# nhcha6/embodied-object-detection

Measured on AMD Instinct MI355X. Metric: frames/sec (640x640, implicit_memory); frames/sec/GPU = value / n_gpus, higher is better.
Workload: dtype f32

## Files before the change

embodied_object_detection_amd/csrc/conv_fp32.hip:

```cpp
#include "conv_operands.h"

namespace eodconv {
namespace {

template <int BM, int BN, int BK, bool TAP4, bool MULTI, int PIPE = 0>
__global__ __launch_bounds__(256) void conv_igemm_kernel(ConvArgs p) {
  constexpr bool BORDER = PIPE == 3;
  static_assert(!BORDER || (BM == 64 && BN == 64 && BK == 32 && !TAP4 && !MULTI), "border-major order: the plain 64x64 kernel");
  constexpr bool PF2 = PIPE == 1;
  constexpr bool DB = PIPE == 2;
  constexpr int LS = BK + 4;
  constexpr int TM = BM / 64, TN = BN / 64;
  constexpr int QPR = BK / 4;
  constexpr int RPP = 256 / QPR;
  constexpr int AR = BM / RPP, BR = BN / RPP;
  static_assert(!TAP4 || BK == 32, "the stem path stages one 7x7 tap per float4: BK must be 32");
  constexpr int BUF = (BM + BN) * LS;
  __shared__ __attribute__((aligned(16))) float lds[(DB ? 2 : 1) * BUF];
  float* As = lds;
  float* Bs = lds + BM * LS;

  const int tid = threadIdx.x;
  const int lane = tid & 63;
  const int wave = tid >> 6;
  const int wm = wave >> 1, wn = wave & 1;

  int M, tile_m, tile_n;
  if constexpr (BORDER) {
    if (!conv_claim_tile_border<BM>(p, M, tile_m, tile_n)) return;
  } else {
    const int t = conv_first_tile<BM>(p, M);
    if (t < 0) return;
    tile_m = t / p.tiles_n;
    tile_n = t - tile_m * p.tiles_n;
  }
  const int m0 = tile_m * BM, n0 = tile_n * BN;
  if (!conv_tile_active(p, m0, BM)) return;
  const int z = blockIdx.y;
  int c_end;
  const int c_begin = conv_chunk_range(p, p.cps, z, c_end);

  const int lr = tid / QPR, lq = tid % QPR;
  int a_off[AR], a_iy[AR], a_ix[AR];
  unsigned a_voff[AR];
  unsigned long long a_mask[AR];
  unsigned a_pitch[MULTI ? AR : 1];
  const int rois = BORDER ? border_rois(p) : 0;
#pragma unroll
  for (int i = 0; i < AR; ++i) {
    const int m = m0 + lr + RPP * i;
    const bool rowok = m < M;
    RowOrigin o;
    if constexpr (BORDER) o = conv_row_origin_border(p, m, rowok, rois);
    else o = conv_row_origin<MULTI>(p, m, rowok);
    a_iy[i] = rowok ? o.iy0 : -(1 << 28);
    a_ix[i] = o.ix0;
    a_off[i] = o.off;
    if (!TAP4) conv_row_address<MULTI>(p, o, rowok, lq, a_voff[i], a_mask[i], a_pitch[MULTI ? i : 0]);
  }
  unsigned w_voff[BR];
#pragma unroll
  for (int j = 0; j < BR; ++j) w_voff[j] = conv_w_row_offset(p, n0 + lr + RPP * j, lq);
  const __amdgpu_buffer_rsrc_t rsrc_x = conv_buffer(p.x, p.x_bytes);
  const __amdgpu_buffer_rsrc_t rsrc_w = conv_buffer(p.w, p.w_bytes);

  unsigned live = 0;
  if constexpr (BORDER) {
    unsigned mine = 0;
#pragma unroll
// ... 87 lines not shown
  auto stage_and_multiply = [&](auto& ar, auto& br, int next_chunk) {
#pragma unroll
    for (int i = 0; i < AR; ++i) *reinterpret_cast<f32x4*>(As + (lr + RPP * i) * LS + 4 * lq) = ar[i];
#pragma unroll
    for (int j = 0; j < BR; ++j) *reinterpret_cast<f32x4*>(Bs + (lr + RPP * j) * LS + 4 * lq) = br[j];
    __syncthreads();
    if (next_chunk < c_end) load_chunk(next_chunk, ar, br);
    if constexpr (TM * TN == 1) {
      f32x4 af[2], bf[2];
      af[0] = *reinterpret_cast<const f32x4*>(a_base);
      bf[0] = *reinterpret_cast<const f32x4*>(b_base);
#pragma unroll
      for (int kk = 0; kk < BK / 8; ++kk) {
        const int cur = kk & 1, nxt = cur ^ 1;
        if (kk + 1 < BK / 8) {
          af[nxt] = *reinterpret_cast<const f32x4*>(a_base + (kk + 1) * 8);
          bf[nxt] = *reinterpret_cast<const f32x4*>(b_base + (kk + 1) * 8);
        }
        __builtin_amdgcn_s_setprio(1);
#pragma unroll
        for (int tt = 0; tt < 4; ++tt)
          if (tt & 1)
            acc_b = __builtin_amdgcn_mfma_f32_32x32x2f32(af[cur][tt], bf[cur][tt], acc_b, 0, 0, 0);
          else
            acc[0][0] = __builtin_amdgcn_mfma_f32_32x32x2f32(af[cur][tt], bf[cur][tt], acc[0][0], 0, 0, 0);
        __builtin_amdgcn_s_setprio(0);
      }
    } else {
      multiply(a_base, b_base);
    }
    __syncthreads();
  };
  load_chunk(c_begin, ar0, br0);
  if constexpr (DB) {
    auto store_tiles = [&](int buf) {
#pragma unroll
      for (int i = 0; i < AR; ++i) *reinterpret_cast<f32x4*>(As + buf * BUF + (lr + RPP * i) * LS + 4 * lq) = ar0[i];
#pragma unroll
      for (int j = 0; j < BR; ++j) *reinterpret_cast<f32x4*>(Bs + buf * BUF + (lr + RPP * j) * LS + 4 * lq) = br0[j];
    };
    store_tiles(0);
    __syncthreads();
    int cur = 0;
    for (int chunk = c_begin; chunk < c_end; ++chunk) {
      const bool more = chunk + 1 < c_end;
      if (more) load_chunk(chunk + 1, ar0, br0);
      multiply(a_base + cur * BUF, b_base + cur * BUF);
      if (more) store_tiles(cur ^ 1);
      __syncthreads();
      cur ^= 1;
    }
  } else if constexpr (PF2) {
    if (c_begin + 1 < c_end) load_chunk(c_begin + 1, ar1, br1);
    for (int chunk = c_begin; chunk < c_end; chunk += 2) {
      stage_and_multiply(ar0, br0, chunk + 2);
      if (chunk + 1 < c_end) stage_and_multiply(ar1, br1, chunk + 3);
    }
  } else {
    for (int chunk = c_begin; chunk < c_end; ++chunk) stage_and_multiply(ar0, br0, chunk + 1);
  }

  if (TM * TN == 1) {
#pragma unroll
    for (int r = 0; r < 16; ++r) acc[0][0][r] += acc_b[r];
  }
  if constexpr (BM == 64 && BN == 256) {
    if (p.out_mode == 2) {
      float sred[16];
#pragma unroll
      for (int r = 0; r < 16; ++r) sred[r] = 0.f;
#pragma unroll
      for (int j = 0; j < TN; ++j) {
        const int co = (wn * TN + j) * 32 + (lane & 31);
        const float bw = p.bias ? p.bias[co] : 0.f;
        const float pw = p.fuse_w[co];
#pragma unroll
        for (int r = 0; r < 16; ++r) {
          float v = (acc[0][j][r] + bw) * p.out_scale;
          if (p.relu) v = fmaxf(v, 0.f);
          sred[r] += v * pw;
        }
      }
#pragma unroll
      for (int off = 16; off > 0; off >>= 1)
#pragma unroll
        for (int r = 0; r < 16; ++r) sred[r] += __shfl_xor(sred[r], off, 64);
      float* red = lds;
      if ((lane & 31) == 0) {
        const int half = lane >> 5;
#pragma unroll
        for (int r = 0; r < 16; ++r) red[(wm * 2 + wn) * 32 + (r & 3) + 8 * (r >> 2) + 4 * half] = sred[r];
      }
      __syncthreads();
      if (tid < BM) {
        const int wr = tid >> 5, rr = tid & 31;
        const float v = red[(wr * 2 + 0) * 32 + rr] + red[(wr * 2 + 1) * 32 + rr] + p.fuse_b;
        const int m = m0 + tid;
        if (m < M) {
          const int tq = (int)fdiv((unsigned)m, p.div_ow);
          const int ox = m - tq * p.OW;
          const int img = (int)fdiv((unsigned)tq, p.div_oh);
          const int oy = tq - img * p.OH;
          const int unit = p.out_units ? p.out_units[img] : img;
          const int dy = tile_n >> 1, dx = tile_n & 1;
          p.y[((size_t)unit * 2 * p.OH + 2 * oy + dy) * (2 * p.OW) + 2 * ox + dx] = eod_sigmoid_precise(v);
        }
      }
      return;
    }
  }
  store_wave_tiles<TM, TN, BM == 64 && BN == 64, BORDER>(p, acc, m0 + wm * TM * 32, n0 + wn * TN * 32, M, z, lane);
}


template <int NW, bool MULTI>
__global__ __launch_bounds__(NW * 64) void conv_wavek_kernel(ConvArgs p) {
  constexpr int BK = 32;
  constexpr int LS = BK + 4;
  constexpr int AR = 4;
  __shared__ __attribute__((aligned(16))) float lds[NW * 2 * 32 * LS];
  const int tid = threadIdx.x;
  const int lane = tid & 63;
  const int wave = tid >> 6;
  float* As = lds + wave * (2 * 32 * LS);
  float* Bs = As + 32 * LS;

  int M;
  const int t = conv_first_tile<32>(p, M);
  if (t < 0) return;
  const int tile_m = t / p.tiles_n;
  const int tile_n = t - tile_m * p.tiles_n;
  const int m0 = tile_m * 32, n0 = tile_n * 32;
  if (!conv_tile_active(p, m0, 32)) return;

  int c_end;
  const int c_begin = conv_chunk_range(p, (p.nchunks + NW - 1) / NW, wave, c_end);

  const int lr = lane >> 3, lq = lane & 7;
  unsigned a_voff[AR];
// ... 86 lines not shown
}

template <int BM, int BN>
static void launch_fp32_tile(const ConvArgs& a, bool tap4, int bk, dim3 grid, hipStream_t s, int dyn) {
  if (tap4)
    hipLaunchKernelGGL((conv_igemm_kernel<BM, BN, 32, true, false>), grid, dim3(256), dyn, s, a);
  else if (a.nlv > 0 && bk == 64)
    hipLaunchKernelGGL((conv_igemm_kernel<BM, BN, 64, false, true>), grid, dim3(256), dyn, s, a);
  else if (a.nlv > 0)
    hipLaunchKernelGGL((conv_igemm_kernel<BM, BN, 32, false, true>), grid, dim3(256), dyn, s, a);
  else if (bk == 64)
    hipLaunchKernelGGL((conv_igemm_kernel<BM, BN, 64, false, false>), grid, dim3(256), dyn, s, a);
  else
    hipLaunchKernelGGL((conv_igemm_kernel<BM, BN, 32, false, false>), grid, dim3(256), dyn, s, a);
}

void launch_conv_fp32(const ConvArgs& a, int tile, int bk, bool tap4, dim3 grid, hipStream_t s, int lds_reserve, int prefetch2) {
  const int dyn = lds_reserve > 0 ? lds_reserve : 0;
  if (a.border) {
    hipLaunchKernelGGL((conv_igemm_kernel<64, 64, 32, false, false, 3>), grid, dim3(256), dyn, s, a);
    return;
  }
  if (prefetch2 == 1 && !tap4 && a.nlv == 0 && bk == 32 && tile == 3) {
    hipLaunchKernelGGL((conv_igemm_kernel<64, 64, 32, false, false, 1>), grid, dim3(256), dyn, s, a);
    return;
  }
  if (prefetch2 == 2 && !tap4 && bk == 32 && tile == 3) {
    if (a.nlv > 0) hipLaunchKernelGGL((conv_igemm_kernel<64, 64, 32, false, true, 2>), grid, dim3(256), dyn, s, a);
    else hipLaunchKernelGGL((conv_igemm_kernel<64, 64, 32, false, false, 2>), grid, dim3(256), dyn, s, a);
    return;
  }
  switch (tile) {
    case 5: hipLaunchKernelGGL((conv_igemm_kernel<64, 256, 32, false, false>), grid, dim3(256), dyn, s, a); break;
    case 1: launch_fp32_tile<128, 128>(a, tap4, bk, grid, s, dyn); break;
    case 2: launch_fp32_tile<128, 64>(a, tap4, bk, grid, s, dyn); break;
    default: launch_fp32_tile<64, 64>(a, tap4, bk, grid, s, dyn); break;
  }
}

void launch_conv_wavek(const ConvArgs& a, int nw, dim3 grid, hipStream_t s) {
  if (a.nlv > 0) {
    if (nw == 8) hipLaunchKernelGGL((conv_wavek_kernel<8, true>), grid, dim3(512), 0, s, a);
    else hipLaunchKernelGGL((conv_wavek_kernel<4, true>), grid, dim3(256), 0, s, a);
  } else {
    if (nw == 8) hipLaunchKernelGGL((conv_wavek_kernel<8, false>), grid, dim3(512), 0, s, a);
    else hipLaunchKernelGGL((conv_wavek_kernel<4, false>), grid, dim3(256), 0, s, a);
  }
}

}
```

embodied_object_detection_amd/csrc/conv_igemm.hip:

```cpp
#include "conv_common.h"
#include "../../include/eod_hip.h"
#include <atomic>
#include <cstdlib>
#include <cstring>

namespace {

using namespace eodconv;

template <int VEC>
__global__ __launch_bounds__(256) void conv_splitk_reduce_kernel(ConvArgs p) {
  EOD_CHAIN_PRIO();
  const int M = conv_row_limit(p, p.M);
  const unsigned per_row = (unsigned)p.Cout / VEC;
  const unsigned total = (unsigned)M * per_row;
  const size_t slab = (size_t)p.M * p.Cout;
  for (unsigned idx = blockIdx.x * blockDim.x + threadIdx.x; idx < total; idx += gridDim.x * blockDim.x) {
    const unsigned m = fdiv(idx, p.div_row);
    if (!conv_row_active(p, (int)m)) continue;
    const unsigned n = (idx - m * per_row) * VEC;
    const float* src = p.partial + (size_t)m * p.Cout + n;
    if (VEC == 4) {
      f32x4 v = {0.f, 0.f, 0.f, 0.f};
      for (int zb = 0; zb < p.splitk; zb += 4) {
// ... 67 lines not shown
    red[sub][col / cpg4][0] = s;
    red[sub][col / cpg4][1] = q;
  }
  __syncthreads();
  if ((int)threadIdx.x < p.gn_groups) {
    double ts = 0.0, tq = 0.0;
    for (int u = 0; u < nsub; ++u) {
      ts += red[u][threadIdx.x][0];
      tq += red[u][threadIdx.x][1];
    }
    p.gn_partial[((size_t)blockIdx.x * p.gn_groups + threadIdx.x) * 2 + 0] = ts;
    p.gn_partial[((size_t)blockIdx.x * p.gn_groups + threadIdx.x) * 2 + 1] = tq;
  }
}

std::atomic<int>& math_mode() {
  static std::atomic<int> v([] {
    const char* e = getenv("EOD_CONV_MATH");
    if (e && strcmp(e, "bf16x3") == 0) return EOD_MATH_BF16X3;
    if (e && strcmp(e, "f16") == 0) return EOD_MATH_F16;
    return EOD_MATH_FP32;
  }());
  return v;
}

struct Plan {
  int tile;
  int bk;
  int glds;
  int bm, bn, tiles_m, tiles_n, splitk, cps, nchunks;
  int wavek;
  int pw_np;
  int border;
};

constexpr int kForcePointwise = 30;

int effective_math(const EodConvDesc* d) { return d->math > 0 ? d->math - 1 : math_mode().load(std::memory_order_relaxed); }

bool pointwise_eligible(const EodConvDesc* d) {
  return effective_math(d) == EOD_MATH_FP32 && d->KH == 1 && d->KW == 1 && d->stride == 1 && d->pad == 0 && d->levels <= 0 && !d->tap4 &&
         d->Cin == d->Kpad && (d->Cin == 64 || d->Cin == 128 || d->Cin == 256) && d->Cout % 64 == 0 && d->out_mode == 0 &&
         (d->res_mode == 0 || d->res_mode == 1) && !d->in_relu && !d->gate && !d->m_count && d->split_n == 0 && !d->gn_partial &&
         d->lds_reserve == 0;
}

constexpr int kForceBorder = 43;
constexpr bool kBorderAuto = true;

bool border_eligible(const EodConvDesc* d) {
  return effective_math(d) == EOD_MATH_FP32 && d->KH == 3 && d->KW == 3 && d->stride == 1 && d->pad == 1 && d->levels <= 0 && !d->tap4 &&
         d->m_count && d->m_segments <= 1 && d->m_unit == d->OH * d->OW && d->OH >= 3 && d->OW >= 3 && d->Cin % 32 == 0 &&
         d->out_mode == 0 && d->res_mode == 0 && !d->in_relu && !d->gate && d->split_n == 0 && !d->gn_partial && d->prefetch2 == 0;
}

Plan make_plan(const EodConvDesc* d, int M) {
  static const int cfg[5][2] = {{128, 128}, {128, 64}, {64, 64}, {256, 128}, {64, 256}};
  Plan pl{};
  int pick = 2;
  const int ft = d->force_tile % 10, fbk = d->force_tile / 10;
  const bool half_ok = !d->tap4 && !d->in_relu;
  const bool f16_forced = (fbk == 8 || fbk == 9) && half_ok;
  if (f16_forced) pick = ft == 4 ? 3 : 2;
  else if (ft >= 1 && ft <= 3) pick = ft - 1;
  else if (ft == 4 && fbk == 5 && half_ok) pick = 3;
  const bool bk64_ok = !d->tap4 && d->Cin % 64 == 0 && d->Kpad % 64 == 0;
  pl.glds = f16_forced ? 3 : ((fbk == 5 && half_ok) ? 2 : 0);
  const int Mp = (d->plan_rows > 0 && d->plan_rows < M) ? d->plan_rows : M;
  const int math = effective_math(d);
  if (d->force_tile == 0 && math == EOD_MATH_F16 && half_ok) {
    pl.glds = 3;
    pick = (long)((Mp + 255) / 256) * ((d->Cout + 127) / 128) >= 256 ? 3 : 2;
  }
  if (d->force_tile == 0 && math == EOD_MATH_BF16X3 && half_ok) {
    pl.glds = 2;
    const long t128 = (long)((Mp + 127) / 128) * ((d->Cout + 127) / 128);
    const long t256 = (long)((Mp + 255) / 256) * ((d->Cout + 127) / 128);
    pick = t256 >= 256 ? 3 : (t128 >= 512 ? 0 : 2);
  }
  if (d->out_mode == 2) {
    pick = 4;
    pl.glds = 0;
  }
  if (d->gate) {
    const bool f16_gated = d->math == EOD_MATH_F16 + 1 && half_ok && d->levels <= 0 && (d->force_tile == 0 || f16_forced);
    pick = 2;
    pl.glds = f16_gated ? 3 : 0;
  }
  if (pl.glds == 3) pl.bk = (fbk == 8 && d->Cin % 64 == 0) ? 64 : 32;
  else pl.bk = (pl.glds == 0 && d->out_mode != 2 && fbk == 2 && bk64_ok) ? 64 : 32;
  const int nchunks = d->Kpad / pl.bk;
  pl.nchunks = nchunks;
  pl.tile = pick + 1;
  pl.bm = cfg[pick][0];
  pl.bn = cfg[pick][1];
  pl.tiles_m = (M + pl.bm - 1) / pl.bm;
  pl.tiles_n = (d->Cout + pl.bn - 1) / pl.bn;
  const long tiles = (long)((Mp + pl.bm - 1) / pl.bm) * pl.tiles_n;
  int splitk = 1;
  if (d->out_mode == 2) {
    splitk = 1;
  } else if (d->force_splitk > 0) {
    splitk = d->force_splitk;
  } else if (pl.glds == 0 && !d->tap4 && nchunks >= 8 &&
             ((d->force_tile == 6 || d->force_tile == 7) ||
              (tiles < 256 && nchunks <= 192 && pl.bk == 32 && d->force_tile == 0 &&
               ((Mp <= 512 && nchunks / (nchunks >= 64 ? 8 : 4) >= 8) || nchunks >= 128)))) {
    pl.wavek = d->force_tile == 6 ? 4 : (d->force_tile == 7 ? 8 : (nchunks >= 64 ? 8 : 4));
    pl.bk = 32;
    pl.nchunks = d->Kpad / 32;
    pl.bm = pl.bn = 32;
    pl.tiles_m = (M + 31) / 32;
    pl.tiles_n = (d->Cout + 31) / 32;
  } else if (tiles < 256 && nchunks >= 8) {
    const int target = (nchunks >= 128 && Mp <= 512) ? 1792 : 512;
    int want = (int)((target + tiles - 1) / tiles);
    int maxs = nchunks / 4;
    splitk = want < maxs ? want : maxs;
    if (splitk < 1) splitk = 1;
  } else if (tiles >= 256 && tiles <= 1024 && d->m_count == nullptr && nchunks >= 18) {
    double best = 1e30;
    for (int sct = 1; sct <= 4; ++sct) {
      if (nchunks / sct < 9) break;
      const double est = (double)((tiles * sct + 255) / 256) / sct + (sct > 1 ? 0.12 : 0.0);
      if (est < best - 1e-9) {
        best = est;
        splitk = sct;
      }
    }
  }
// ... 62 lines not shown
    if (d->OW != (d->W + 2 * d->pad - d->KW) / d->stride + 1) return EOD_ERR_BAD_DIMS;
  }
  if (d->levels <= 0 && (long)d->N * d->H * d->W * d->Cin >= (1L << 29)) return EOD_ERR_BAD_DIMS;
  if ((long)d->Cout * d->Kpad >= (1L << 29)) return EOD_ERR_BAD_DIMS;
  if (d->KH * d->KW > 64) return EOD_ERR_BAD_DIMS;
  if ((long)total_rows(d) * (d->Cout > d->Cin ? d->Cout : d->Cin) >= (1L << 31)) return EOD_ERR_BAD_DIMS;
  if (d->out_mode == 1 && (d->Cout % 4 != 0)) return EOD_ERR_BAD_DIMS;
  if (d->out_mode == 2) {
    if (d->Cout != 1024 || d->KH != 1 || d->KW != 1 || d->stride != 1 || d->tap4 || d->levels > 0 || d->res_mode != 0 || d->in_relu ||
        d->force_splitk > 1)
      return EOD_ERR_BAD_DIMS;
    if (!d->fuse_w) return EOD_ERR_NULL;
  }
  if (d->out_mode < 0 || d->out_mode > 2) return EOD_ERR_BAD_DIMS;
  if (d->res_mode != 0 && !d->res) return EOD_ERR_NULL;
  if (d->res_mode == 2 && ((d->OH & 1) || (d->OW & 1))) return EOD_ERR_BAD_DIMS;
  if (d->m_count && d->m_unit <= 0) return EOD_ERR_BAD_DIMS;
  if (d->m_segments > 1) {
    if (!d->m_count || d->levels > 0 || d->out_mode == 2 || d->m_segments > EOD_MAX_BATCH || d->N % d->m_segments != 0)
      return EOD_ERR_BAD_DIMS;
    if (((long)(d->N / d->m_segments) * d->OH * d->OW) % d->m_unit != 0) return EOD_ERR_BAD_DIMS;
  }
  if (d->gate && (d->out_mode != 0 || d->split_n != 0 || d->gn_partial)) return EOD_ERR_BAD_DIMS;
  if (d->gate && d->force_tile != 0 && d->force_tile % 10 != 3 && d->force_tile != 6 && d->force_tile != 7) return EOD_ERR_BAD_DIMS;
  if (d->gate && d->force_tile / 10 == 5) return EOD_ERR_BAD_DIMS;
  if (d->gate && (d->force_tile / 10 == 8 || d->force_tile / 10 == 9) &&
      (d->math != EOD_MATH_F16 + 1 || d->force_tile % 10 != 3 || d->levels > 0 || d->tap4 || d->in_relu))
    return EOD_ERR_BAD_DIMS;
  if (d->math < 0 || d->math > EOD_MATH_F16 + 1) return EOD_ERR_BAD_DIMS;
  if ((d->force_tile / 10 == 8 || d->force_tile / 10 == 9) && d->force_tile % 10 != 3 && d->force_tile % 10 != 4) return EOD_ERR_BAD_DIMS;
  if (d->lds_reserve < 0 || d->lds_reserve > 48 * 1024) return EOD_ERR_BAD_DIMS;
  if (d->force_tile == kForcePointwise && (!pointwise_eligible(d) || d->force_splitk > 1)) return EOD_ERR_BAD_DIMS;
  if (d->force_tile == kForceBorder && (!border_eligible(d) || d->force_splitk > 1)) return EOD_ERR_BAD_DIMS;
  if (d->split_n != 0) {
    if (!d->y2) return EOD_ERR_NULL;
    if (d->split_n < 0 || d->split_n >= d->Cout || d->out_mode != 0 || d->res_mode != 0 || d->levels > 0 || d->gn_partial)
      return EOD_ERR_BAD_DIMS;
  }
  if (d->gn_partial) {
    const int cpg = d->gn_groups > 0 ? d->Cout / d->gn_groups : 0;
    if (d->levels <= 0 || d->m_count || d->out_mode != 0 || d->gn_groups <= 0 || d->gn_groups > 64 || d->Cout % d->gn_groups != 0 ||
        cpg > 64 || (cpg & (cpg - 1)) != 0 || cpg < 4 || d->Cout % 4 != 0 || d->Cout > 1024 || 256 % (d->Cout / 4) != 0 ||
        64 % (cpg / 4) != 0)
      return EOD_ERR_BAD_DIMS;
  }
  if (!eod_aligned16(d->x) || !eod_aligned16(d->w) || !eod_aligned16(d->w_split) || !eod_aligned16(d->w_half)) return EOD_ERR_ALIGN;
  return EOD_OK;
}

}

extern "C" int eod_set_conv_math(int mode) {
  if (mode != EOD_MATH_FP32 && mode != EOD_MATH_BF16X3 && mode != EOD_MATH_F16) return EOD_ERR_BAD_DIMS;
  return math_mode().exchange(mode);
}

extern "C" int eod_get_conv_math(void) { return math_mode().load(); }

extern "C" size_t eod_conv_split_weights_bytes(int Cout, int Kpad) {
  return (Cout > 0 && Kpad > 0 && Kpad % 32 == 0) ? (size_t)Cout * Kpad * 6 : 0;
}

extern "C" int eod_conv_split_weights_bf16x3(const float* w, int Cout, int Kpad, void* out, eod_stream_t stream) {
  if (!w || !out) return EOD_ERR_NULL;
  if (Cout <= 0 || Kpad <= 0 || Kpad % 32 != 0 || (long)Cout * Kpad * 6 >= (1L << 32)) return EOD_ERR_BAD_DIMS;
  if (!eod_aligned16(w) || !eod_aligned16(out)) return EOD_ERR_ALIGN;
// ... 70 lines not shown
    a.w3_bytes = (unsigned)((size_t)d->Cout * d->Kpad * 6);
    a.wh = d->w_half;
    a.wh_bytes = (unsigned)((size_t)d->Cout * d->Kpad * 2);
  }
  a.nlv = d->levels > 0 ? d->levels : 0;
  for (int l = 0; l < a.nlv; ++l) {
    a.lv_off[l] = d->level_off[l];
    a.lv_h[l] = d->level_h[l];
    a.lv_w[l] = d->level_w[l];
  }
  if (a.nlv) a.lv_off[a.nlv] = d->level_off[a.nlv];
  a.relu = d->relu; a.res_mode = d->res_mode; a.in_relu = d->in_relu; a.out_mode = d->out_mode;
  a.gate = d->gate;
  a.out_scale = d->out_scale;
  a.gn_partial = d->gn_partial;
  a.gn_groups = d->gn_groups;
  a.y2 = d->y2;
  a.split_n = d->split_n;
  const Plan pl = make_plan(d, a.M);
  if (d->gn_partial && pl.splitk <= 1) return EOD_ERR_BAD_DIMS;
  a.nchunks = pl.nchunks;
  a.splitk = pl.splitk; a.cps = pl.cps; a.tiles_m = pl.tiles_m; a.tiles_n = pl.tiles_n;
  a.border = pl.border;
  if (pl.splitk > 1) {
    const size_t need = (size_t)pl.splitk * a.M * a.Cout * sizeof(float);
    if (!d->workspace || d->workspace_bytes < need) return EOD_ERR_CAPACITY;
  }
  dim3 grid(pl.tiles_m * pl.tiles_n, pl.splitk);
  if (pl.border) grid.x = (pl.tiles_m + 7) / 8 * 8 * pl.tiles_n;
  if (pl.pw_np) launch_conv_pointwise(a, pl.pw_np, grid, s);
  else if (pl.wavek) launch_conv_wavek(a, pl.wavek, grid, s);
  else if (pl.glds == 3) launch_conv_f16(a, pl.tile, pl.bk, grid, s);
  else if (pl.glds == 2) launch_conv_bf16x3(a, pl.tile, grid, s);
  else launch_conv_fp32(a, pl.tile, pl.bk, d->tap4 != 0, grid, s, d->lds_reserve, d->prefetch2);
  if (pl.splitk > 1) {
    const size_t total = (size_t)a.M * a.Cout;
    const bool vec = a.Cout % 4 == 0;
    int blocks = (int)((total / (vec ? 4 : 1) + 255) / 256);
    if (blocks > 2048) blocks = 2048;
    if (blocks < 1) blocks = 1;
    if (a.gn_partial) {
      int chunks = 0;
      for (int l = 0; l < a.nlv; ++l) chunks += (a.lv_off[l + 1] - a.lv_off[l] + EOD_GN_ROWS - 1) / EOD_GN_ROWS;
      hipLaunchKernelGGL(conv_splitk_reduce_gn_kernel, dim3(chunks), dim3(256), 0, s, a);
    } else if (vec) hipLaunchKernelGGL(conv_splitk_reduce_kernel<4>, dim3(blocks), dim3(256), 0, s, a);
    else hipLaunchKernelGGL(conv_splitk_reduce_kernel<1>, dim3(blocks), dim3(256), 0, s, a);
  }
  return eod_launch_status();
}
```

embodied_object_detection_amd/modeling/roi_heads.py:

```python
from __future__ import annotations

from typing import Dict, List, Tuple

import torch

from .. import ops
from ..registry import ROI_HEADS_REGISTRY


RESULT_SETS = 3


class RoiBuffers:

    def __init__(self, heads: "DeticCascadeROIHeads", B: int, lockstep: bool):
        R, D, dev = heads.R, heads.topk, heads.device
        f32 = dict(dtype=torch.float32, device=dev)
        self.device, self.B, self.R, self.D, self.rows = dev, B, R, D, B * R
        self.lockstep = lockstep
        self.batch, self.m_segments = (B, B) if lockstep else (1, 0)
        self.plan_like_single = True
        self.pool7 = torch.empty((B * R, 7, 7, 256), **f32)
        self.h1 = torch.empty((B * R, 1, 1, 1024), **f32)
        self.h2 = torch.empty((B * R, 1, 1, 1024), **f32)
# ... 82 lines not shown
        self.stages = []
        for k in range(self.num_stages):
            fc1_w = sd[f"roi_heads.box_head.{k}.fc1.weight"]
            fc1_w = fc1_w.view(-1, 256, 7, 7).permute(0, 2, 3, 1).reshape(fc1_w.shape[0], -1, 1, 1).contiguous()
            p = f"roi_heads.box_predictor.{k}"
            st = dict(
                fc1=ops.Conv(fc1_w, sd[f"roi_heads.box_head.{k}.fc1.bias"], device=device, name=f"box_head.{k}.fc1"),
                fc2=ops.Conv(sd[f"roi_heads.box_head.{k}.fc2.weight"][:, :, None, None], sd[f"roi_heads.box_head.{k}.fc2.bias"],
                             device=device, name=f"box_head.{k}.fc2"),
                cls=ops.Conv(sd[f"{p}.cls_score.linear.weight"][:, :, None, None], sd[f"{p}.cls_score.linear.bias"], device=device,
                             name=f"box_predictor.{k}.cls_score.linear"),
                bb0=ops.Conv(sd[f"{p}.bbox_pred.0.weight"][:, :, None, None], sd[f"{p}.bbox_pred.0.bias"], device=device,
                             name=f"box_predictor.{k}.bbox_pred.0"),
                bb2=ops.Conv(sd[f"{p}.bbox_pred.2.weight"][:, :, None, None], sd[f"{p}.bbox_pred.2.bias"], device=device,
                             name=f"box_predictor.{k}.bbox_pred.2"),
                zs=sd[f"{p}.cls_score.zs_weight"].contiguous().to(device),
            )
            st["cls_bb0"] = ops.Conv(torch.cat([sd[f"{p}.cls_score.linear.weight"], sd[f"{p}.bbox_pred.0.weight"]], dim=0)[:, :, None, None],
                                     torch.cat([sd[f"{p}.cls_score.linear.bias"], sd[f"{p}.bbox_pred.0.bias"]], dim=0), device=device,
                                     name=f"box_predictor.{k}.cls_score.linear+bbox_pred.0")
            assert st["zs"].shape == (512, self.C1), (st["zs"].shape, self.C1)
            self.stages.append(st)
        m = "roi_heads.mask_head"
        self.mask_convs = [ops.Conv(sd[f"{m}.mask_fcn{i}.weight"], sd[f"{m}.mask_fcn{i}.bias"], pad=1, device=device, name=f"mask_fcn{i}")
                           for i in range(1, 5)]
        for conv in self.mask_convs:
            conv.prefetch2 = int(__import__("os").environ.get("EOD_MASK_PREFETCH2", "0"))
        self.deconv = ops.Conv(sd[f"{m}.deconv.weight"], sd[f"{m}.deconv.bias"], device=device, deconv=True, name="mask_deconv")
        self.pred_w = sd[f"{m}.predictor.weight"].reshape(-1).contiguous().to(device)
        self.pred_b = float(sd[f"{m}.predictor.bias"].item())
        self.bufs = RoiBuffers(self, 1, lockstep=False)
        self.bufs.expose_on(self)
        self.fuse_mask_tail = True
        self.merge_cls_bb0 = True
        self.fuse_stage_tail = True
        self.fold_deltas = False
        self.graph_cascade = False
        self._graphs = {}
        self.det_pass_lds_reserve = int(__import__("os").environ.get("EOD_DET_LDS_RESERVE", "0"))
        self.prop_pass_lds_reserve = int(__import__("os").environ.get("EOD_PROP_LDS_RESERVE", "0"))
        self.selectors = [ops.DetectionSelector(self.R, self.C1, self.topk, device, groups=True) for _ in range(RESULT_SETS)]
        self.selector = self.selectors[0]

    def set_classifier(self, zs: torch.Tensor) -> None:
        zs = zs.to(dtype=torch.float32).contiguous().to(self.device)
        if zs.dim() != 2 or zs.shape[0] != 512 or not 2 <= zs.shape[1] <= ops.ZS_WIDE_MAX_C1:
            raise ValueError(f"classifier matrix {tuple(zs.shape)}: expected [512, C + 1] with 1 <= C <= {ops.ZS_WIDE_MAX_C1 - 1}")
        for st in self.stages:
            st["zs"] = zs
        if zs.shape[1] != self.C1:
            self.C1 = int(zs.shape[1])
            self.num_classes = self.C1 - 1
            self.bufs.set_width(self.C1)
            self.bufs.expose_on(self)
            self.selectors = [ops.DetectionSelector(self.R, self.C1, self.topk, self.device, groups=True) for _ in range(RESULT_SETS)]
            self.selector = self.selectors[0]
        self._graphs = {}

    def forward_box(self, views: List[torch.Tensor], shapes, prop_boxes: torch.Tensor, prop_scores: torch.Tensor, count: torch.Tensor,
                    image_hw: Tuple[int, int], sel: int = 0, mem_rescore=None, after_stage0=None):
        h3, w3 = shapes[0]
        H, W = image_hw
        R = self.R
        if self.graph_cascade:
            key = (views[0].data_ptr(), prop_boxes.data_ptr(), prop_scores.data_ptr(), count.data_ptr(), mem_rescore is not None, H, W)
            gs = self._graphs.get(key)
# ... 68 lines not shown
                after_stage0()
            if not self.merge_cls_bb0:
                st["bb0"](g.h2, rows, 1, 1, relu=True, m_count=count, m_unit=1, out=g.hb, m_segments=segs, plan_rows=pr)
            st["bb2"](g.hb, rows, 1, 1, m_count=count, m_unit=1, out=g.deltas, m_segments=segs, plan_rows=pr)
            if self.fold_deltas and not last:
                pending = self.cascade_weights[k]
            else:
                ops.apply_deltas(g.deltas, 4, boxes, g.boxes[k + 1], count, R, self.cascade_weights[k], not last, float(W), float(H),
                                 batch=batch)
                boxes = g.boxes[k + 1]
        return boxes, pending

    def forward_mask(self, views, shapes, boxes: torch.Tensor, count: torch.Tensor, cap: int, out: torch.Tensor,
                     rows: torch.Tensor = None, bufs=None, lds_reserve: int = 0, tag=None, g: RoiBuffers = None,
                     boxes_per_image: int = 0):
        g = g if g is not None else self.bufs
        h3, w3 = shapes[0]
        mpool, mbuf, mup = bufs if bufs is not None else g.mask_bufs
        if not self.fuse_mask_tail and mup is None:
            raise NotImplementedError("fuse_mask_tail = False: the lock-step buffers hold no deconv output; run the two-launch mask tail "
                                      "on the single-scene model")
        cap, pr = g.B * cap, g.plan_rows(cap * 196)
        ops.roi_align(views[0], views[1], views[2], h3, w3, 256, boxes, count, cap, 14, out=mpool, box_rows=rows, batch=g.batch,
                      boxes_per_image=g.per_scene(boxes_per_image))
        src, dst = mpool, mbuf
        self.deconv.lds_reserve = lds_reserve
        for conv in self.mask_convs:
            conv.lds_reserve = lds_reserve
            conv.event_tag = tag
            conv(src, cap, 14, 14, relu=True, m_count=count, m_unit=196, out=dst, plan_rows=pr)
            src, dst = dst, src
        if self.fuse_mask_tail:
            self.deconv(src, cap, 14, 14, relu=True, m_count=count, m_unit=196, out=out, fuse=(self.pred_w, self.pred_b, rows),
                        plan_rows=pr)
        else:
            self.deconv(src, cap, 14, 14, relu=True, m_count=count, m_unit=196, out=mup, plan_rows=pr)
            ops.mask_predictor_sigmoid(mup, self.pred_w, self.pred_b, cap * 784, 256, count, 784, out=out, out_units=rows)
        return out

    def forward(self, views, shapes, prop_boxes, prop_scores, prop_count, image_hw):
        det = self.forward_box(views, shapes, prop_boxes, prop_scores, prop_count, image_hw)
        det_boxes, det_scores, det_classes, det_rows, det_count = det
        self.forward_mask(views, shapes, det_boxes, det_count, self.topk, self.det_masks)
        return det

    def forward_mask_memory(self, views, shapes, prop_boxes, prop_count, rows: torch.Tensor = None, rows_count: torch.Tensor = None,
                            bufs=None, tag=None, g: RoiBuffers = None, lds_reserve: int = None):
        g = g if g is not None else self.bufs
        lds = self.prop_pass_lds_reserve if lds_reserve is None else lds_reserve
        if rows is not None:
            rows, rows_count = g.roi_list(rows, rows_count, self.R)
            return self.forward_mask(views, shapes, prop_boxes, rows_count, min(self.R, 128), g.prop_masks, rows=rows, bufs=bufs,
                                     lds_reserve=lds, tag=tag, g=g, boxes_per_image=self.R)
        return self.forward_mask(views, shapes, prop_boxes, prop_count, self.R, g.prop_masks, bufs=bufs, lds_reserve=lds, tag=tag, g=g,
                                 boxes_per_image=self.R)

    def detection_masks(self, g: RoiBuffers, views, shapes, sel, slot: int, dedup: bool, lds_reserve: int, tag=None):
        rows, count = g.roi_list(sel.rep_list, sel.rep_count, self.topk, slot) if dedup else g.roi_list(None, sel.count, self.topk, slot)
        return self.forward_mask(views, shapes, sel.boxes, count, self.topk, g.det_masks, rows=rows, lds_reserve=lds_reserve, tag=tag,
                                 g=g, boxes_per_image=self.topk)

    def postprocess_and_paste(self, g: RoiBuffers, sel, post: dict, image_hw, mask_threshold: float, dedup: bool):
        H, W = image_hw
        B, D, dev = g.B, self.topk, self.device
        post["boxes"] = torch.empty((B * D, 4), dtype=torch.float32, device=dev)
        post["scores"] = torch.empty((B * D,), dtype=torch.float32, device=dev)
        post["classes"] = torch.empty((B * D,), dtype=torch.int32, device=dev)
# ... 13 lines not shown
```

embodied_object_detection_amd/ops.py:

```python
from __future__ import annotations

import ctypes as C
from typing import Dict, Optional, Sequence, Tuple

import numpy as np
import torch

from . import _lib
from ._lib import EodConvDesc, EodDetDesc, EodMemWriteDesc, EodProposalDesc, check


_raw_stream = getattr(torch._C, "_cuda_getCurrentRawStream", None)


def _stream() -> int:
    if _raw_stream is not None:
        return _raw_stream(torch.cuda.current_device())
    return torch.cuda.current_stream().cuda_stream


def _ptr(t: Optional[torch.Tensor]) -> Optional[int]:
    return None if t is None else t.data_ptr()


# ... 27 lines not shown
def set_conv_math(mode: str) -> str:
    if mode not in _CONV_MATH:
        hint = ""
        if str(mode).lower() == "fp16":
            hint = (' ("fp16" / FP16 is the config key of autocast training: modeling.training.build_trainer / AmpTrainer, which choose '
                    'the arithmetic per launch; the process-wide inference arithmetic is "f16")')
        raise ValueError(f"conv math must be one of {sorted(_CONV_MATH)}, got {mode!r}{hint}")
    prev = _lib.load().eod_set_conv_math(_CONV_MATH[mode])
    check(min(prev, 0), "eod_set_conv_math")
    return {v: k for k, v in _CONV_MATH.items()}[prev]


def get_conv_math() -> str:
    return {v: k for k, v in _CONV_MATH.items()}[_lib.load().eod_get_conv_math()]


def fold_bn(w: torch.Tensor, bn_w, bn_b, bn_mean, bn_var, eps: float = 1e-5):
    scale = bn_w / torch.sqrt(bn_var + eps)
    return w * scale.view(-1, 1, 1, 1), bn_b - bn_mean * scale


def pack_conv_weight(w_oihw: torch.Tensor, cin_pad: Optional[int] = None) -> Tuple[torch.Tensor, int]:
    O, I, KH, KW = w_oihw.shape
    w = w_oihw.permute(0, 2, 3, 1).contiguous()
    if cin_pad is not None and cin_pad != I:
        wp = torch.zeros((O, KH, KW, cin_pad), dtype=w.dtype)
        wp[..., :I] = w
        w = wp
    K = w.shape[1] * w.shape[2] * w.shape[3]
    Kpad = (K + 31) // 32 * 32
    out = torch.zeros((O, Kpad), dtype=torch.float32)
    out[:, :K] = w.reshape(O, K)
    return out.contiguous(), Kpad


class Conv:

    def __init__(self, w_oihw: torch.Tensor, bias: Optional[torch.Tensor], stride: int = 1, pad: int = 0,
                 device="cuda", cin_pad: Optional[int] = None, deconv: bool = False, name: str = ""):
        self.name = name
        if deconv:
            Cin, Cout, kh, kw = w_oihw.shape
            assert kh == 2 and kw == 2
            w = w_oihw.permute(2, 3, 1, 0).reshape(4 * Cout, Cin, 1, 1).contiguous()
            self.out_mode = 1
            self.KH = self.KW = 1
            self.stride, self.pad = 1, 0
            self.Cin, self.Cout = Cin, 4 * Cout
        else:
            w = w_oihw
            self.out_mode = 0
            self.Cout, cin, self.KH, self.KW = w.shape
            self.Cin = cin_pad or cin
            self.stride, self.pad = stride, pad
        packed, self.Kpad = pack_conv_weight(w, cin_pad)
        self.tap4 = 1 if self.Cin == 4 else 0
        if not self.tap4 and self.Cin % 32 != 0:
            raise ValueError(f"{name}: Cin={self.Cin} must be a multiple of 32 (or 4 for the stem)")
        self.w = packed.to(device)
        self.bias = None if bias is None else bias.detach().to(torch.float32).contiguous().to(device)
        self.desc = EodConvDesc()
        self._lib = _lib.load()
        self.w_split = None
        self.w_half = None
        self.event_log = None
        self.event_tag = None
# ... 1546 lines not shown
```

Before: 324.7.

## Split fused mask-tail deconv into two 128-wide passes per tile

```diff
diff --git a/embodied_object_detection_amd/csrc/conv_fp32.hip b/embodied_object_detection_amd/csrc/conv_fp32.hip
--- a/embodied_object_detection_amd/csrc/conv_fp32.hip
+++ b/embodied_object_detection_amd/csrc/conv_fp32.hip
@@ -2,10 +2,39 @@
 
 namespace eodconv {
 namespace {
+
+__device__ __forceinline__ void tail_chain(const ConvArgs& p, const f32x16& acc, int co, float (&sred)[16]) {
+  const float bw = p.bias ? p.bias[co] : 0.f;
+  const float pw = p.fuse_w[co];
+#pragma unroll
+  for (int r = 0; r < 16; ++r) {
+    float v = (acc[r] + bw) * p.out_scale;
+    if (p.relu) v = fmaxf(v, 0.f);
+    sred[r] = __builtin_fmaf(v, pw, sred[r]);
+  }
+}
+__device__ __forceinline__ void tail_butterfly(float (&sred)[16]) {
+#pragma unroll
+  for (int off = 16; off > 0; off >>= 1)
+#pragma unroll
+    for (int r = 0; r < 16; ++r) sred[r] += __shfl_xor(sred[r], off, 64);
+}
+__device__ __forceinline__ void tail_store(const ConvArgs& p, float v, int m, int tile_n) {
+  const int tq = (int)fdiv((unsigned)m, p.div_ow);
+  const int ox = m - tq * p.OW;
+  const int img = (int)fdiv((unsigned)tq, p.div_oh);
+  const int oy = tq - img * p.OH;
+  const int unit = p.out_units ? p.out_units[img] : img;
+  const int dy = tile_n >> 1, dx = tile_n & 1;
+  p.y[((size_t)unit * 2 * p.OH + 2 * oy + dy) * (2 * p.OW) + 2 * ox + dx] = eod_sigmoid_precise(v);
+}
 
 template <int BM, int BN, int BK, bool TAP4, bool MULTI, int PIPE = 0>
 __global__ __launch_bounds__(256) void conv_igemm_kernel(ConvArgs p) {
   constexpr bool BORDER = PIPE == 3;
+  constexpr bool TAIL2 = BM == 64 && BN == 128;
+  constexpr int NPASS = TAIL2 ? 2 : 1;
+  static_assert(!TAIL2 || (BK == 32 && !TAP4 && !MULTI && PIPE == 0), "two-pass tail: the default pipeline");
   static_assert(!BORDER || (BM == 64 && BN == 64 && BK == 32 && !TAP4 && !MULTI), "border-major order: the plain 64x64 kernel");
   constexpr bool PF2 = PIPE == 1;
   constexpr bool DB = PIPE == 2;
@@ -16,7 +45,8 @@
   constexpr int AR = BM / RPP, BR = BN / RPP;
   static_assert(!TAP4 || BK == 32, "the stem path stages one 7x7 tap per float4: BK must be 32");
   constexpr int BUF = (BM + BN) * LS;
-  __shared__ __attribute__((aligned(16))) float lds[(DB ? 2 : 1) * BUF];
+  constexpr int RED = TAIL2 ? 2 * 2 * 32 : 0;
+  __shared__ __attribute__((aligned(16))) float lds[(DB ? 2 : 1) * BUF + RED];
   float* As = lds;
   float* Bs = lds + BM * LS;
 
@@ -34,7 +64,7 @@
     tile_m = t / p.tiles_n;
     tile_n = t - tile_m * p.tiles_n;
   }
-  const int m0 = tile_m * BM, n0 = tile_n * BN;
+  const int m0 = tile_m * BM, n0 = tile_n * BN * NPASS;
   if (!conv_tile_active(p, m0, BM)) return;
   const int z = blockIdx.y;
   int c_end;
@@ -188,7 +218,53 @@
     __syncthreads();
   };
   load_chunk(c_begin, ar0, br0);
-  if constexpr (DB) {
+  if constexpr (TAIL2) {
+    float* hand = lds;
+    float* red = lds + BUF;
+#pragma nounroll
+    for (int pass = 0; pass < NPASS; ++pass) {
+      for (int chunk = c_begin; chunk < c_end; ++chunk) stage_and_multiply(ar0, br0, chunk + 1);
+      if (pass + 1 < NPASS) {
+#pragma unroll
+        for (int j = 0; j < BR; ++j) w_voff[j] = conv_w_row_offset(p, n0 + (pass + 1) * BN + lr + RPP * j, lq);
+        walk = ChunkWalker<BK, MULTI>(p, c_begin);
+        load_chunk(c_begin, ar0, br0);
+      }
+      float sred[16];
+      if (wn == 0) {
+#pragma unroll
+        for (int r = 0; r < 16; ++r) sred[r] = 0.f;
+#pragma unroll
+        for (int j = 0; j < TN; ++j) tail_chain(p, acc[0][j], pass * BN + j * 32 + (lane & 31), sred);
+#pragma unroll
+        for (int r = 0; r < 16; ++r) hand[(wm * 16 + r) * 64 + lane] = sred[r];
+      }
+      __syncthreads();
+      if (wn == 1) {
+#pragma unroll
+        for (int r = 0; r < 16; ++r) sred[r] = hand[(wm * 16 + r) * 64 + lane];
+#pragma unroll
+        for (int j = 0; j < TN; ++j) tail_chain(p, acc[0][j], pass * BN + (TN + j) * 32 + (lane & 31), sred);
+        tail_butterfly(sred);
+        if ((lane & 31) == 0) {
+          const int half = lane >> 5;
+#pragma unroll
+          for (int r = 0; r < 16; ++r) red[(pass * 2 + wm) * 32 + (r & 3) + 8 * (r >> 2) + 4 * half] = sred[r];
+        }
+      }
+      __syncthreads();
+#pragma unroll
+      for (int j = 0; j < TN; ++j)
+#pragma unroll
+        for (int r = 0; r < 16; ++r) acc[0][j][r] = 0.f;
+    }
+    if (tid < BM) {
+      const int wr = tid >> 5, rr = tid & 31;
+      const float v = red[(0 * 2 + wr) * 32 + rr] + red[(1 * 2 + wr) * 32 + rr] + p.fuse_b;
+      if (m0 + tid < M) tail_store(p, v, m0 + tid, tile_n);
+    }
+    return;
+  } else if constexpr (DB) {
     auto store_tiles = [&](int buf) {
 #pragma unroll
       for (int i = 0; i < AR; ++i) *reinterpret_cast<f32x4*>(As + buf * BUF + (lr + RPP * i) * LS + 4 * lq) = ar0[i];
@@ -226,21 +302,8 @@
 #pragma unroll
       for (int r = 0; r < 16; ++r) sred[r] = 0.f;
 #pragma unroll
-      for (int j = 0; j < TN; ++j) {
-        const int co = (wn * TN + j) * 32 + (lane & 31);
-        const float bw = p.bias ? p.bias[co] : 0.f;
-        const float pw = p.fuse_w[co];
-#pragma unroll
-        for (int r = 0; r < 16; ++r) {
-          float v = (acc[0][j][r] + bw) * p.out_scale;
-          if (p.relu) v = fmaxf(v, 0.f);
-          sred[r] += v * pw;
-        }
-      }
-#pragma unroll
-      for (int off = 16; off > 0; off >>= 1)
-#pragma unroll
-        for (int r = 0; r < 16; ++r) sred[r] += __shfl_xor(sred[r], off, 64);
+      for (int j = 0; j < TN; ++j) tail_chain(p, acc[0][j], (wn * TN + j) * 32 + (lane & 31), sred);
+      tail_butterfly(sred);
       float* red = lds;
       if ((lane & 31) == 0) {
         const int half = lane >> 5;
@@ -251,16 +314,7 @@
       if (tid < BM) {
         const int wr = tid >> 5, rr = tid & 31;
         const float v = red[(wr * 2 + 0) * 32 + rr] + red[(wr * 2 + 1) * 32 + rr] + p.fuse_b;
-        const int m = m0 + tid;
-        if (m < M) {
-          const int tq = (int)fdiv((unsigned)m, p.div_ow);
-          const int ox = m - tq * p.OW;
-          const int img = (int)fdiv((unsigned)tq, p.div_oh);
-          const int oy = tq - img * p.OH;
-          const int unit = p.out_units ? p.out_units[img] : img;
-          const int dy = tile_n >> 1, dx = tile_n & 1;
-          p.y[((size_t)unit * 2 * p.OH + 2 * oy + dy) * (2 * p.OW) + 2 * ox + dx] = eod_sigmoid_precise(v);
-        }
+        if (m0 + tid < M) tail_store(p, v, m0 + tid, tile_n);
       }
       return;
     }
@@ -413,6 +467,7 @@
   }
   switch (tile) {
     case 5: hipLaunchKernelGGL((conv_igemm_kernel<64, 256, 32, false, false>), grid, dim3(256), dyn, s, a); break;
+    case 7: hipLaunchKernelGGL((conv_igemm_kernel<64, 128, 32, false, false>), grid, dim3(256), dyn, s, a); break;
     case 1: launch_fp32_tile<128, 128>(a, tap4, bk, grid, s, dyn); break;
     case 2: launch_fp32_tile<128, 64>(a, tap4, bk, grid, s, dyn); break;
     default: launch_fp32_tile<64, 64>(a, tap4, bk, grid, s, dyn); break;
diff --git a/embodied_object_detection_amd/csrc/conv_igemm.hip b/embodied_object_detection_amd/csrc/conv_igemm.hip
--- a/embodied_object_detection_amd/csrc/conv_igemm.hip
+++ b/embodied_object_detection_amd/csrc/conv_igemm.hip
@@ -123,6 +123,7 @@
   int wavek;
   int pw_np;
   int border;
+  int tail2;
 };
 
 constexpr int kForcePointwise = 30;
@@ -138,6 +139,8 @@
 
 constexpr int kForceBorder = 43;
 constexpr bool kBorderAuto = true;
+
+constexpr int kForceTailWide = 45;
 
 bool border_eligible(const EodConvDesc* d) {
   return effective_math(d) == EOD_MATH_FP32 && d->KH == 3 && d->KW == 3 && d->stride == 1 && d->pad == 1 && d->levels <= 0 && !d->tap4 &&
@@ -187,6 +190,10 @@
   pl.bn = cfg[pick][1];
   pl.tiles_m = (M + pl.bm - 1) / pl.bm;
   pl.tiles_n = (d->Cout + pl.bn - 1) / pl.bn;
+  if (d->out_mode == 2 && d->force_tile != kForceTailWide) {
+    pl.tail2 = 1;
+    pl.bn = 128;
+  }
   const long tiles = (long)((Mp + pl.bm - 1) / pl.bm) * pl.tiles_n;
   int splitk = 1;
   if (d->out_mode == 2) {
@@ -315,6 +322,7 @@
   if (d->lds_reserve < 0 || d->lds_reserve > 48 * 1024) return EOD_ERR_BAD_DIMS;
   if (d->force_tile == kForcePointwise && (!pointwise_eligible(d) || d->force_splitk > 1)) return EOD_ERR_BAD_DIMS;
   if (d->force_tile == kForceBorder && (!border_eligible(d) || d->force_splitk > 1)) return EOD_ERR_BAD_DIMS;
+  if (d->force_tile == kForceTailWide && d->out_mode != 2) return EOD_ERR_BAD_DIMS;
   if (d->split_n != 0) {
     if (!d->y2) return EOD_ERR_NULL;
     if (d->split_n < 0 || d->split_n >= d->Cout || d->out_mode != 0 || d->res_mode != 0 || d->levels > 0 || d->gn_partial)
@@ -451,7 +459,7 @@
   else if (pl.wavek) launch_conv_wavek(a, pl.wavek, grid, s);
   else if (pl.glds == 3) launch_conv_f16(a, pl.tile, pl.bk, grid, s);
   else if (pl.glds == 2) launch_conv_bf16x3(a, pl.tile, grid, s);
-  else launch_conv_fp32(a, pl.tile, pl.bk, d->tap4 != 0, grid, s, d->lds_reserve, d->prefetch2);
+  else launch_conv_fp32(a, pl.tail2 ? 7 : pl.tile, pl.bk, d->tap4 != 0, grid, s, d->lds_reserve, d->prefetch2);
   if (pl.splitk > 1) {
     const size_t total = (size_t)a.M * a.Cout;
     const bool vec = a.Cout % 4 == 0;
diff --git a/embodied_object_detection_amd/modeling/roi_heads.py b/embodied_object_detection_amd/modeling/roi_heads.py
--- a/embodied_object_detection_amd/modeling/roi_heads.py
+++ b/embodied_object_detection_amd/modeling/roi_heads.py
@@ -138,6 +138,7 @@
         self.bufs = RoiBuffers(self, 1, lockstep=False)
         self.bufs.expose_on(self)
         self.fuse_mask_tail = True
+        self.mask_tail_force_tile = 0
         self.merge_cls_bb0 = True
         self.fuse_stage_tail = True
         self.fold_deltas = False
@@ -272,7 +273,7 @@
             src, dst = dst, src
         if self.fuse_mask_tail:
             self.deconv(src, cap, 14, 14, relu=True, m_count=count, m_unit=196, out=out, fuse=(self.pred_w, self.pred_b, rows),
-                        plan_rows=pr)
+                        plan_rows=pr, force_tile=self.mask_tail_force_tile)
         else:
             self.deconv(src, cap, 14, 14, relu=True, m_count=count, m_unit=196, out=mup, plan_rows=pr)
             ops.mask_predictor_sigmoid(mup, self.pred_w, self.pred_b, cap * 784, 256, count, 784, out=out, out_units=rows)
diff --git a/embodied_object_detection_amd/ops.py b/embodied_object_detection_amd/ops.py
--- a/embodied_object_detection_amd/ops.py
+++ b/embodied_object_detection_amd/ops.py
@@ -83,6 +83,9 @@
     out = torch.zeros((O, Kpad), dtype=torch.float32)
     out[:, :K] = w.reshape(O, K)
     return out.contiguous(), Kpad
+
+
+FORCE_TAIL_WIDE = 45
 
 
 class Conv:
```

New measurement: 324.4, median of 2. No clear change (-0.1%).
